# codex-storage/codex-storage-proofs-circuits

Hardware: AMD Instinct MI355X
Metric: Poseidon2-BN254 permutations/sec per GPU; full proof-input witnesses/sec (higher is better)
Workload: dtype u32x9 (29-bit limbs, Montgomery mod BN254 r)

## Files before the change

### codex-storage-proofs-circuits_amd/csrc/internal.hpp

```cpp
#pragma once
#include <hip/hip_runtime.h>

#include <sys/resource.h>
#include <sys/syscall.h>
#include <unistd.h>

#include <condition_variable>
#include <cstdint>
#include <deque>
#include <functional>
#include <memory>
#include <mutex>
#include <string>
#include <thread>
#include <vector>

#include "../../include/codex_p2.h"
#include "workers.hpp"

namespace cp2i {

bool env_decimal(const char* name, uint64_t* value, bool* set);
bool env_keep_trees(int* mode);
size_t mem_limit_bytes();
// ... 135 lines not shown
  void* p = nullptr;
  size_t bytes = 0;
  cp2_ctx* owner = nullptr;
  cp2_ctx* home = nullptr;
  bool borrowed = false;
  DevBuf() = default;
  DevBuf(const DevBuf&) = delete;
  DevBuf& operator=(const DevBuf&) = delete;
  ~DevBuf() { release(); }
  void borrow(void* q, size_t n) {
    release();
    p = q;
    bytes = n;
    borrowed = true;
  }
  void release() {
    if (p && !borrowed) {
      if (owner && owner->stuck) {
      } else if (owner) {
        (void)hipStreamSynchronize(owner->stream);
        if (owner->aux_stream) (void)hipStreamSynchronize(owner->aux_stream);
        if (owner->aux2_stream) (void)hipStreamSynchronize(owner->aux2_stream);
        owner->pool->put(false, p, bytes);
      } else if (!(home && home->stuck)) {
        dev_free(p, bytes);
      }
    }
    p = nullptr;
    bytes = 0;
    owner = nullptr;
    home = nullptr;
    borrowed = false;
  }
  int alloc(cp2_ctx* ctx, size_t n) {
    release();
    if (n == 0) n = 16;
    hipError_t e = dev_malloc(&p, n);
    if (e != hipSuccess) {
      (void)hipGetLastError();
      ctx->pool->trim();
      e = dev_malloc(&p, n);
    }
    if (e != hipSuccess) {
      (void)hipGetLastError();
      p = nullptr;
      ctx->err = std::string("hipMalloc(") + std::to_string(n) + "): " + hipGetErrorString(e);
      return CP2_ERR_ALLOC;
    }
    bytes = n;
    home = ctx;
    return CP2_OK;
  }
  int scratch(cp2_ctx* ctx, size_t n) {
    release();
    size_t got = 0;
    p = ctx->pool->get(false, n, &got);
    if (!p) {
      ctx->err = std::string("device scratch of ") + std::to_string(n) + " bytes: allocation failed";
      return CP2_ERR_ALLOC;
    }
    bytes = got;
    owner = ctx;
    return CP2_OK;
  }
  uint8_t* u8() const { return static_cast<uint8_t*>(p); }
};
// ... 55 lines not shown
```

### codex-storage-proofs-circuits_amd/csrc/proof_many.cpp

```cpp
#include <hip/hip_runtime.h>

#include <fcntl.h>
#include <unistd.h>

#include <algorithm>
#include <cstring>
#include <map>
#include <memory>
#include <string>
#include <vector>

#include "dataset_obj.hpp"
#include "proof_input_obj.hpp"
#include "trees.hpp"

using namespace cp2i;

namespace {

struct Req {
  cp2_dataset* ds = nullptr;
  uint64_t slot = 0;
  uint8_t entropy[32];
  size_t at = 0;
  size_t id = 0;
};

int refuse(cp2_ctx* ctx, size_t i, const std::string& why) {
  ctx->err = "request " + std::to_string(i) + ": " + why;
  return CP2_ERR_INVALID;
}

size_t depth_of(size_t n) { return layer_sizes_of(n).size() - 1; }

bool same_circuit(const cp2_config& a, const cp2_config& b) {
  return a.max_depth == b.max_depth && a.max_log2_nslots == b.max_log2_nslots && a.cell_size == b.cell_size && a.block_size == b.block_size &&
         a.n_samples == b.n_samples;
}

int validate(cp2_ctx* ctx, cp2_dataset* const* ds, const uint64_t* slot_idx, size_t n) {
  for (size_t i = 0; i < n; ++i) {
    const cp2_dataset* d = ds[i];
    if (!d) return refuse(ctx, i, "NULL dataset");
    if (d->ctx != ctx) return refuse(ctx, i, "its dataset belongs to another context");
    const cp2_config& c = d->cfg;
// ... 17 lines not shown
  }
  return CP2_OK;
}

int check_roots(cp2_ctx* ctx, cp2_dataset* const* ds, const uint64_t* slot_idx, size_t n) {
  std::vector<uint64_t> a(n);
  for (size_t i = 0; i < n; ++i)
    a[i] = (uint64_t)reinterpret_cast<uintptr_t>(dataset_roots_dev(ds[i])) + (slot_idx[i] - ds[i]->first_slot) * 32;
  std::vector<uint8_t> got(n * 32);
  DevBuf d_a, d_r;
  CP2_TRY(d_a.scratch(ctx, n * 8));
  CP2_TRY(d_r.scratch(ctx, n * 32));
  CP2_HIP(ctx, hipMemcpyAsync(d_a.p, a.data(), n * 8, hipMemcpyHostToDevice, ctx->stream));
  CP2_HIP(ctx, cp2k::launch_gather_addr(static_cast<const uint64_t*>(d_a.p), n, 32, d_r.p, ctx->stream));
  CP2_HIP(ctx, hipMemcpyAsync(got.data(), d_r.p, n * 32, hipMemcpyDeviceToHost, ctx->stream));
  CP2_HIP(ctx, hipStreamSynchronize(ctx->stream));
  for (size_t i = 0; i < n; ++i)
    if (std::memcmp(&got[i * 32], &ds[i]->dlayers[slot_idx[i] * 32], 32) != 0)
      return refuse(ctx, i, "the root its dataset tree holds for slot " + std::to_string(slot_idx[i]) +
                                " (cp2_dataset_set_roots) differs from the slot's built root");
  return CP2_OK;
}

int prepare(cp2_ctx* ctx, cp2_dataset* const* ds, const uint64_t* slot_idx, size_t n) {
  CP2_TRY(validate(ctx, ds, slot_idx, n));
  CP2_HIP(ctx, hipSetDevice(ctx->device));
  for (size_t i = 0; i < n; ++i)
    if (!ds[i]->have_roots) CP2_TRY(cp2_dataset_set_roots(ds[i], nullptr));
  return check_roots(ctx, ds, slot_idx, n);
}

std::string who(bool named, const Req* r) { return named ? "request " + std::to_string(r->id) + ": " : std::string(); }

int run_pass(cp2_ctx* ctx, const std::vector<const Req*>& rq, size_t n_rf, size_t n_rfile, size_t n_cf, bool named, cp2_proof_input** out) {
  const size_t n = rq.size(), nr = n_rf + n_rfile;
  const cp2_config& c0 = rq[0]->ds->cfg;
  const size_t ns = c0.n_samples, md = (size_t)c0.max_depth, cs = c0.cell_size, bs = c0.block_size, cpb = bs / cs;
  const size_t T = n * ns, R = nr * ns, C = T - R, RF = n_rf * ns, CF = n_cf * ns;
  auto store = std::make_shared<BatchStore>();
  if (T) {
    std::vector<cp2k::ManyReq> reqs(n);
    std::vector<cp2k::TreeGeom> geoms;
    std::map<std::string, uint32_t> geom_of;
    for (size_t j = 0; j < n; ++j) {
      const cp2_dataset* ds = rq[j]->ds;
      cp2k::ManyReq& q = reqs[j];
      std::memset(&q, 0, sizeof q);
      std::memcpy(q.entropy, rq[j]->entropy, 32);
      std::memcpy(q.slot_root, &ds->dlayers[rq[j]->slot * 32], 32);
      q.n_cells = ds->cfg.n_cells;
      q.cpb = cpb;
      if (j < nr) {
        cp2k::TreeGeom g;
        std::memset(&g, 0, sizeof g);
        trees_geom(ds->trees, &g);
        auto it = geom_of.emplace(std::string(reinterpret_cast<const char*>(&g), sizeof g), (uint32_t)geoms.size());
        if (it.second) geoms.push_back(g);
        q.geom = it.first->second;
        q.nodes = (uint64_t)reinterpret_cast<uintptr_t>(ds->trees->nodes.p);
        q.slot = rq[j]->slot - ds->first_slot;
      }
    }
    std::vector<uint64_t> blk(C), gen, cpaths, ctail, ccell;
    std::vector<uint8_t> checks(2 * C * 32);
    PinBuf h_blocks;
    const size_t rows = T * md + T + 2 * C;
    DevBuf d_req, d_geom, d_idx, d_blk, d_addr, d_rows, d_cells, d_gen, d_caddr;
    CP2_TRY(d_req.scratch(ctx, n * sizeof(cp2k::ManyReq)));
    CP2_TRY(d_geom.scratch(ctx, std::max<size_t>(1, geoms.size()) * sizeof(cp2k::TreeGeom)));
    CP2_TRY(d_idx.scratch(ctx, T * 8));
    CP2_TRY(d_blk.scratch(ctx, T * 8));
    CP2_TRY(d_addr.scratch(ctx, rows * 8));
    CP2_TRY(d_rows.scratch(ctx, rows * 32));
    CP2_TRY(d_cells.scratch(ctx, (C * cpb + T) * cs));
    CP2_TRY(store->idx.alloc(ctx, T * 8));
    CP2_TRY(store->paths.alloc(ctx, T * md * 32));
    CP2_TRY(store->leaves.alloc(ctx, T * 32));
    CP2_TRY(store->cells.alloc(ctx, T * cs));
    uint8_t* cells_out = d_cells.u8() + C * cpb * cs;
    uint64_t* addr = static_cast<uint64_t*>(d_addr.p);
    CP2_HIP(ctx, hipMemcpyAsync(d_req.p, reqs.data(), n * sizeof(cp2k::ManyReq), hipMemcpyHostToDevice, ctx->stream));
    if (!geoms.empty())
      CP2_HIP(ctx, hipMemcpyAsync(d_geom.p, geoms.data(), geoms.size() * sizeof(cp2k::TreeGeom), hipMemcpyHostToDevice, ctx->stream));
    CP2_HIP(ctx, cp2k::launch_sample_many(static_cast<const cp2k::ManyReq*>(d_req.p), static_cast<const cp2k::TreeGeom*>(d_geom.p), n,
                                          (uint32_t)ns, (uint32_t)md, static_cast<uint64_t*>(d_idx.p), static_cast<uint64_t*>(d_blk.p), addr,
                                          ctx->stream));
    CP2_HIP(ctx, hipMemcpyAsync(store->idx.p, d_idx.p, T * 8, hipMemcpyDeviceToHost, ctx->stream));
    if (C) CP2_HIP(ctx, hipMemcpyAsync(blk.data(), static_cast<uint64_t*>(d_blk.p) + R, C * 8, hipMemcpyDeviceToHost, ctx->stream));
    CP2_HIP(ctx, hipStreamSynchronize(ctx->stream));
    const uint64_t* idx = static_cast<const uint64_t*>(store->idx.p);

    gen.assign((CF + RF) * 2, 0);
    uint64_t* seeds = gen.data();
    uint64_t* firsts = seeds + CF + RF;
    for (size_t q = 0; q < CF; ++q) {
      const Req* r = rq[nr + q / ns];
      seeds[q] = cp2_slot_seed(r->ds->cfg.seed, r->slot);
      firsts[q] = blk[q] * cpb;
    }
    for (size_t p = 0; p < RF; ++p) {
      const Req* r = rq[p / ns];
      seeds[CF + p] = cp2_slot_seed(r->ds->cfg.seed, r->slot);
      firsts[CF + p] = idx[p];
    }
    if (CF + RF) {
      CP2_TRY(d_gen.scratch(ctx, gen.size() * 8));
      const uint64_t* dg = static_cast<const uint64_t*>(d_gen.p);
      CP2_HIP(ctx, hipMemcpyAsync(d_gen.p, gen.data(), gen.size() * 8, hipMemcpyHostToDevice, ctx->stream));
      CP2_HIP(ctx, cp2k::launch_gen_fake_cells_many(dg, dg + CF + RF, cpb, CF * cpb, cs, d_cells.p, ctx->stream));
      CP2_HIP(ctx, cp2k::launch_gen_fake_cells_many(dg + CF, dg + CF + RF + CF, 1, RF, cs, cells_out, ctx->stream));
    }
    if (C > CF) {
      const size_t n_req_file = (C - CF) / ns;
      CP2_TRY(h_blocks.alloc(ctx, (C - CF) * bs));
      std::vector<std::string> failed(fill_threads(ctx));
      on_threads(fill_threads(ctx), n_req_file, [&](int w, size_t k) {
        const size_t q0 = CF + k * ns;
        const Req* r = rq[nr + q0 / ns];
        const std::string fname = slot_file_name(r->ds->file_base, r->slot);
        const int fd = open(fname.c_str(), O_RDONLY);
        if (fd < 0) { failed[w] = who(named, r) + "slot " + std::to_string(r->slot) + ": " + slot_file_error(fname, 0); return false; }
        int err = 0;
        size_t c = 0;
        for (; c < ns && !err; ++c) err = slot_file_read_rest(fd, h_blocks.u8() + (q0 - CF + c) * bs, bs, blk[q0 + c] * bs);
        close(fd);
        if (err) {
          failed[w] = who(named, r) + "block " + std::to_string(blk[q0 + c - 1]) + " of slot " + std::to_string(r->slot) +
                      ": " + slot_file_error(fname, err);
          return false;
        }
        return true;
      });
      for (const auto& f : failed)
        if (!f.empty()) { ctx->err = f; return CP2_ERR_IO; }
      CP2_HIP(ctx, hipMemcpyAsync(d_cells.u8() + CF * bs, h_blocks.p, (C - CF) * bs, hipMemcpyHostToDevice, ctx->stream));
    }
    cp2_slot_trees* mini = nullptr;
    struct Mini { cp2_slot_trees*& t; ~Mini() { cp2_slot_trees_free(t); } } mini_guard{mini};
    if (C) {
      cpaths.assign(C * md, 0);
      ctail.assign(3 * C, 0);
      ccell.assign(C, 0);
      CP2_TRY(cp2_slot_trees_build_dev(ctx, d_cells.p, C, cs, bs, cpb, &mini));
      const size_t depth_b = depth_of(cpb);
      const uint64_t mb = (uint64_t)reinterpret_cast<uintptr_t>(mini->nodes.p);
      std::vector<uint64_t> rr(depth_b + 1);
      for (size_t q = 0; q < C; ++q) {
        const Req* r = rq[nr + q / ns];
        const cp2_dataset* ds = r->ds;
        const uint64_t ls = r->slot - ds->first_slot, cell = idx[R + q], b = blk[q], in_block = cell % cpb;
        const uint64_t kb = (uint64_t)reinterpret_cast<uintptr_t>(ds->compact.p);
        uint64_t* P = &cpaths[q * md];
        path_rows(mini, q, in_block, depth_b + 1, rr.data());
        for (size_t d = 0; d < depth_b; ++d) P[d] = rr[d] == NO_ROW ? 0 : mb + rr[d] * 32;
        uint64_t j = b, m = ds->cfg.n_cells / cpb;
        for (size_t d = 0; d + 1 < ds->csizes.size(); ++d) {
          const uint64_t sib = j ^ 1;
          P[depth_b + d] = sib < m ? kb + (ds->coff[d] + ls * ds->csizes[d] + sib) * 32 : 0;
          j >>= 1;
          m = (m + 1) >> 1;
        }
        ctail[q] = mb + (q * cpb + in_block) * 32;
        ctail[C + 2 * q] = kb + (ds->coff[0] + ls * ds->csizes[0] + b) * 32;
        ctail[C + 2 * q + 1] = mb + (mini->toff[0] + q) * 32;
        ccell[q] = (uint64_t)reinterpret_cast<uintptr_t>(d_cells.u8()) + (q * cpb + in_block) * cs;
      }
      CP2_TRY(d_caddr.scratch(ctx, C * 8));
      CP2_HIP(ctx, hipMemcpyAsync(addr + R * md, cpaths.data(), C * md * 8, hipMemcpyHostToDevice, ctx->stream));
      CP2_HIP(ctx, hipMemcpyAsync(addr + T * md + R, ctail.data(), 3 * C * 8, hipMemcpyHostToDevice, ctx->stream));
      CP2_HIP(ctx, hipMemcpyAsync(d_caddr.p, ccell.data(), C * 8, hipMemcpyHostToDevice, ctx->stream));
      CP2_HIP(ctx, cp2k::launch_gather_addr(static_cast<const uint64_t*>(d_caddr.p), C, cs, cells_out + R * cs, ctx->stream));
    }
    CP2_HIP(ctx, cp2k::launch_gather_addr(addr, rows, 32, d_rows.p, ctx->stream));
    CP2_HIP(ctx, hipMemcpyAsync(store->paths.p, d_rows.p, T * md * 32, hipMemcpyDeviceToHost, ctx->stream));
    CP2_HIP(ctx, hipMemcpyAsync(store->leaves.p, d_rows.u8() + T * md * 32, T * 32, hipMemcpyDeviceToHost, ctx->stream));
    if (C) CP2_HIP(ctx, hipMemcpyAsync(checks.data(), d_rows.u8() + (T * md + T) * 32, 2 * C * 32, hipMemcpyDeviceToHost, ctx->stream));
    CP2_HIP(ctx, hipMemcpyAsync(store->cells.p, cells_out, T * cs, hipMemcpyDeviceToHost, ctx->stream));
    CP2_HIP(ctx, hipStreamSynchronize(ctx->stream));
    for (size_t q = 0; q < C; ++q)
      if (std::memcmp(&checks[2 * q * 32], &checks[(2 * q + 1) * 32], 32) != 0) {
        const Req* r = rq[nr + q / ns];
        ctx->err = who(named, r) + "block " + std::to_string(blk[q]) + " of slot " + std::to_string(r->slot) +
                   " does not hash to its stored root (slot data changed since the build?)";
        return CP2_ERR_IO;
      }
    if (R > RF) {
      std::vector<std::string> failed(fill_threads(ctx));
      on_threads(fill_threads(ctx), n_rfile, [&](int w, size_t k) {
        const Req* r = rq[n_rf + k];
        const std::string fname = slot_file_name(r->ds->file_base, r->slot);
        const int fd = open(fname.c_str(), O_RDONLY);
        if (fd < 0) { failed[w] = who(named, r) + slot_file_error(fname, 0); return false; }
        int err = 0;
        const size_t p0 = (n_rf + k) * ns;
        for (size_t c = 0; c < ns && !err; ++c) err = read_file_cell(fd, cs, idx[p0 + c], store->cells.u8() + (p0 + c) * cs);
        close(fd);
        if (err) { failed[w] = who(named, r) + slot_file_error(fname, err); return false; }
        return true;
      });
      for (const auto& f : failed)
        if (!f.empty()) { ctx->err = f; return CP2_ERR_IO; }
    }
  }
  std::vector<ProofItem> items(n);
  for (size_t j = 0; j < n; ++j) items[j] = {rq[j]->ds, rq[j]->slot, rq[j]->entropy, &out[rq[j]->at]};
  return proof_inputs_from_store(items.data(), n, store, store->cells.u8());
}

}

int cp2i::prove_requests(cp2_ctx* ctx, cp2_dataset* const* ds, const uint64_t* slot_idx, const uint8_t* entropies, size_t n, size_t at0,
                         bool named, cp2_proof_input** out) {
  for (size_t i = 0; i < n; ++i) out[i] = nullptr;
  if (n == 0) return CP2_OK;
  CP2_HIP(ctx, hipSetDevice(ctx->device));
  std::vector<Req> req(n);
  std::vector<const Req*> res_fake, res_file, cmp_fake, cmp_file, roots_only;
  for (size_t i = 0; i < n; ++i) {
    req[i].ds = ds[i];
    req[i].slot = slot_idx[i];
    req[i].at = i;
    req[i].id = at0 + i;
    canonical_felt(entropies + 32 * i, req[i].entropy);
    const cp2_dataset* d = ds[i];
    (d->trees ? (d->from_file ? res_file : res_fake) : d->tree_mode == 2 ? (d->from_file ? cmp_file : cmp_fake) : roots_only).push_back(&req[i]);
  }
  auto fail = [&](int st) {
    for (size_t i = 0; i < n; ++i) { cp2_proof_input_free(out[i]); out[i] = nullptr; }
    return st;
  };
  for (const Req* r : roots_only) {
    const int st = cp2_proof_inputs_generate_batch(r->ds, &r->slot, 1, r->entropy, &out[r->at]);
    if (st != CP2_OK) {
      ctx->err = who(named, r) + ctx->err;
      return fail(st);
    }
  }
  const cp2_config& c0 = ds[0]->cfg;
  const size_t per_req = std::max<size_t>(1, (size_t)c0.n_samples * c0.block_size);
  const size_t chunk = std::max<size_t>(1, ctx->stage_bytes / per_req);
  std::vector<const Req*> compact(cmp_fake);
  compact.insert(compact.end(), cmp_file.begin(), cmp_file.end());
  const size_t n_res = res_fake.size() + res_file.size();
  size_t c = 0;
  for (bool first = true; first ? n_res + compact.size() > 0 : c < compact.size(); first = false) {
    std::vector<const Req*> rq;
    if (first) {
      rq = res_fake;
      rq.insert(rq.end(), res_file.begin(), res_file.end());
    }
    const size_t c1 = std::min(compact.size(), c + chunk);
    rq.insert(rq.end(), compact.begin() + (long)c, compact.begin() + (long)c1);
    const size_t n_cf = c < cmp_fake.size() ? std::min(c1, cmp_fake.size()) - c : 0;
    const int st = run_pass(ctx, rq, first ? res_fake.size() : 0, first ? res_file.size() : 0, n_cf, named, out);
    if (st != CP2_OK) return fail(st);
    c = c1;
  }
  return CP2_OK;
}

extern "C" int cp2_proof_inputs_generate_many(cp2_ctx* ctx, cp2_dataset* const* ds, const uint64_t* slot_idx, const uint8_t* entropies, size_t n,
                                              cp2_proof_input** out) try {
  if (!ctx) return CP2_ERR_INVALID;
  if (n && (!ds || !slot_idx || !entropies || !out)) {
    ctx->err = "cp2_proof_inputs_generate_many: NULL array";
    return CP2_ERR_INVALID;
  }
  for (size_t i = 0; i < n; ++i) out[i] = nullptr;
  if (n == 0) return CP2_OK;
  CP2_REFUSE_STUCK(ctx);
  CP2_TRY(prepare(ctx, ds, slot_idx, n));
  return prove_requests(ctx, ds, slot_idx, entropies, n, 0, true, out);
} catch (const std::bad_alloc&) {
  return CP2_ERR_ALLOC;
} catch (...) {
  return CP2_ERR_INVALID;
}

extern "C" int cp2_proof_inputs_export_many(cp2_ctx* ctx, cp2_dataset* const* ds, const uint64_t* slot_idx, const uint8_t* entropies, size_t n,
                                            const char* const* paths, int threads, size_t batch, uint64_t* total_bytes) try {
  if (!ctx) return CP2_ERR_INVALID;
  if (n && (!ds || !slot_idx || !entropies)) {
    ctx->err = "cp2_proof_inputs_export_many: NULL array";
    return CP2_ERR_INVALID;
  }
  if (total_bytes) *total_bytes = 0;
  if (n == 0) return CP2_OK;
  CP2_REFUSE_STUCK(ctx);
  CP2_TRY(prepare(ctx, ds, slot_idx, n));
  if (batch == 0) batch = 512;
// ... 38 lines not shown
```

### codex-storage-proofs-circuits_amd/csrc/slot_trees.cpp

```cpp
#include <hip/hip_runtime.h>

#include <fcntl.h>
#include <sys/mman.h>
#include <sys/stat.h>
#include <unistd.h>

#include <algorithm>
#include <atomic>
#include <chrono>
#include <condition_variable>
#include <cstdio>
#include <cstdlib>
#include <cstring>
#include <memory>
#include <mutex>
#include <new>
#include <string>
#include <vector>

#include "trees.hpp"
#include "checksum64.hpp"
#include "fake_turns.hpp"
#include "ingest_turns.hpp"
#include "fill_pipeline.hpp"
// ... 17 lines not shown
}

int aux_stream(cp2_ctx* ctx, hipStream_t* out, int which) {
  hipStream_t& st = which == 2 ? ctx->aux2_stream : ctx->aux_stream;
  if (!st) CP2_HIP(ctx, hipStreamCreateWithFlags(&st, hipStreamNonBlocking));
  *out = st;
  return CP2_OK;
}

std::string slot_file_name(const std::string& base, uint64_t slot) { return fill_slot_file_name(base, slot); }

int trees_check_geometry(size_t cell_size, size_t block_size, size_t n_cells, size_t n_slots) {
  if (cell_size == 0 || block_size == 0 || n_cells == 0 || n_slots == 0) return CP2_ERR_INVALID;
  if (block_size % cell_size != 0) return CP2_ERR_INVALID;
  size_t cpb = block_size / cell_size;
  if (n_cells % cpb != 0) return CP2_ERR_INVALID;
  if (cell_size > ((size_t)1 << 30) || n_cells > ((size_t)1 << 40) || n_slots > ((size_t)1 << 32)) return CP2_ERR_INVALID;
  if ((unsigned __int128)n_cells * n_slots > ((unsigned __int128)1 << 44)) return CP2_ERR_INVALID;
  return CP2_OK;
}

}

cp2i::BuildScratch::~BuildScratch() {
  if (!ctx) return;
  (void)hipSetDevice(ctx->device);
  (void)hipStreamSynchronize(ctx->stream);
  if (ctx->aux_stream) (void)hipStreamSynchronize(ctx->aux_stream);
  if (ctx->aux2_stream) (void)hipStreamSynchronize(ctx->aux2_stream);
}

static int trees_layout(cp2_slot_trees* t, cp2i::DevBuf* borrow_from = nullptr) {
  t->bsizes = layer_sizes_of(t->cpb);
  t->tsizes = layer_sizes_of(t->nblocks);
  if (t->bsizes.size() > (size_t)cp2k::TreeGeom::MAX_LAYERS || t->tsizes.size() > (size_t)cp2k::TreeGeom::MAX_LAYERS) return CP2_ERR_INVALID;
  size_t off = 0;
  t->boff.clear();
  t->toff.clear();
  const size_t nb = t->n_slots * t->nblocks;
  for (size_t k = 0; k < t->bsizes.size(); ++k) {
    t->boff.push_back(off);
    if (k + 1 < t->bsizes.size()) off += nb * t->bsizes[k];
  }
  for (size_t k = 0; k < t->tsizes.size(); ++k) {
    t->toff.push_back(off);
    off += t->n_slots * t->tsizes[k];
  }
  if (borrow_from) {
    if (borrow_from->bytes < off * 32) CP2_TRY(borrow_from->scratch(t->ctx, off * 32));
    t->nodes.borrow(borrow_from->p, off * 32);
    return CP2_OK;
  }
  return t->pooled_nodes ? t->nodes.scratch(t->ctx, off * 32) : t->nodes.alloc(t->ctx, off * 32);
}

size_t cp2i::trees_node_bytes(size_t n_slots, size_t cell_size, size_t block_size, size_t n_cells) {
  const size_t cpb = block_size / cell_size, nblocks = n_cells / cpb;
  size_t per_block = 0, per_slot = 0;
  const std::vector<size_t> b = layer_sizes_of(cpb), t = layer_sizes_of(nblocks);
  for (size_t k = 0; k + 1 < b.size(); ++k) per_block += b[k];
  for (size_t m : t) per_slot += m;
  return n_slots * (nblocks * per_block + per_slot) * 32;
}

void cp2i::trees_geom(const cp2_slot_trees* t, cp2k::TreeGeom* g) {
  std::memset(g, 0, sizeof *g);
  g->nb = (uint32_t)t->bsizes.size();
  g->nt = (uint32_t)t->tsizes.size();
  g->cpb = t->cpb;
  g->nblocks = t->nblocks;
  g->n_cells = t->n_cells;
  for (size_t k = 0; k < t->bsizes.size(); ++k) { g->boff[k] = t->boff[k]; g->bsz[k] = t->bsizes[k]; }
  for (size_t k = 0; k < t->tsizes.size(); ++k) { g->toff[k] = t->toff[k]; g->tsz[k] = t->tsizes[k]; }
}

static cp2_slot_trees* trees_new(cp2_ctx* ctx, size_t n_slots, size_t cell_size, size_t block_size, size_t n_cells) {
  cp2_slot_trees* t = new (std::nothrow) cp2_slot_trees();
  if (!t) return nullptr;
  t->ctx = ctx;
  t->n_slots = n_slots;
  t->cell_size = cell_size;
  t->block_size = block_size;
  t->n_cells = n_cells;
  t->cpb = block_size / cell_size;
  t->nblocks = n_cells / t->cpb;
  return t;
}

static int trees_build_layers(cp2_slot_trees* t, size_t s0, size_t s1, hipStream_t st) {
  cp2_ctx* ctx = t->ctx;
  uint8_t* base = t->nodes.u8();
  const size_t ns = s1 - s0, nb = ns * t->nblocks;
  for (size_t k = 0; k + 1 < t->bsizes.size(); ++k)
    CP2_HIP(ctx, cp2k::launch_compress_layer(base + (t->boff[k] + s0 * t->nblocks * t->bsizes[k]) * 32,
                                             base + (t->boff[k + 1] + s0 * t->nblocks * t->bsizes[k + 1]) * 32, t->bsizes[k], nb,
// ... 141 lines not shown
namespace {
bool unit_geometry_ok(uint64_t units_per_slot, size_t cell_size, size_t block_size, size_t cells_per_unit) {
  if (!is_pow2(units_per_slot) || cell_size == 0 || block_size < cell_size) return false;
  const size_t nb = cells_per_unit / (block_size / cell_size);
  return nb >= 2 && is_pow2(nb);
}
}
extern "C" int cp2_slot_trees_build_fake_units(cp2_ctx* ctx, uint64_t dataset_seed, uint64_t units_per_slot, uint64_t first_unit,
                                               size_t n_units, size_t cell_size, size_t block_size, size_t cells_per_unit,
                                               cp2_slot_trees** out) try {
  if (!ctx || !out || units_per_slot == 0) return CP2_ERR_INVALID;
  CP2_TRY(trees_check_geometry(cell_size, block_size, cells_per_unit, n_units));
  if (units_per_slot > 1 && !unit_geometry_ok(units_per_slot, cell_size, block_size, cells_per_unit)) return CP2_ERR_INVALID;
  return trees_build_fake(ctx, dataset_seed, first_unit, n_units, cell_size, block_size, cells_per_unit, 0, nullptr, out, units_per_slot);
} catch (const std::bad_alloc&) {
  return CP2_ERR_ALLOC;
} catch (...) {
  return CP2_ERR_INVALID;
}

extern "C" int cp2_slot_trees_build_file_units(cp2_ctx* ctx, const char* file_base, uint64_t units_per_slot, uint64_t first_unit,
                                               size_t n_units, size_t cell_size, size_t block_size, size_t cells_per_unit,
                                               cp2_slot_trees** out) try {
  if (!ctx || !out || !file_base || units_per_slot == 0 || cell_size > SLOT_FILE_MAX_CELL) return CP2_ERR_INVALID;
  CP2_TRY(trees_check_geometry(cell_size, block_size, cells_per_unit, n_units));
  if (units_per_slot > 1 && !unit_geometry_ok(units_per_slot, cell_size, block_size, cells_per_unit)) return CP2_ERR_INVALID;
  return trees_build_files(ctx, file_base, first_unit, n_units, cell_size, block_size, cells_per_unit, 0, nullptr, out, units_per_slot);
} catch (const std::bad_alloc&) {
  return CP2_ERR_ALLOC;
} catch (...) {
  return CP2_ERR_INVALID;
}

extern "C" int cp2_slot_trees_build_dev(cp2_ctx* ctx, const void* d_cells, size_t n_slots, size_t cell_size,
                                        size_t block_size, size_t n_cells, cp2_slot_trees** out) try {
  if (!ctx || !out || !d_cells) return CP2_ERR_INVALID;
  *out = nullptr;
  CP2_REFUSE_STUCK(ctx);
  CP2_TRY(trees_check_geometry(cell_size, block_size, n_cells, n_slots));
  CP2_HIP(ctx, hipSetDevice(ctx->device));
  std::unique_ptr<cp2_slot_trees> t(trees_new(ctx, n_slots, cell_size, block_size, n_cells));
  if (!t) return CP2_ERR_ALLOC;
  t->src = CellSrc::Dev;
  t->d_cells = static_cast<const uint8_t*>(d_cells);
  CP2_TRY(trees_layout(t.get()));
  CP2_HIP(ctx, cp2k::launch_hash_cells(d_cells, cell_size, n_slots * n_cells, t->nodes.p, ctx->stream));
  CP2_TRY(trees_build_layers(t.get(), 0, n_slots, ctx->stream));
  *out = t.release();
  return CP2_OK;
} catch (const std::bad_alloc&) {
  return CP2_ERR_ALLOC;
} catch (...) {
  return CP2_ERR_INVALID;
}

namespace {

size_t env_size(const char* name, size_t dflt) {
  const char* v = std::getenv(name);
  if (!v || !*v) return dflt;
  char* end = nullptr;
  unsigned long long x = std::strtoull(v, &end, 10);
  return (end && *end == 0 && x > 0) ? (size_t)x : dflt;
}

struct IngestPipe {
  static constexpr int MAX_DEPTH = 8;
  static constexpr size_t DIRECT_ALIGN = 4096;
  size_t cell_multiple = 1;
  cp2_ctx* ctx = nullptr;
  hipStream_t copy = nullptr;
  int pin_depth = 0, dev_depth = 0;
  PinBuf pinned[MAX_DEPTH];
  DevBuf dev[MAX_DEPTH];
  hipEvent_t copied[MAX_DEPTH] = {};
  hipEvent_t uploaded[MAX_DEPTH] = {};
  hipEvent_t hashed[MAX_DEPTH] = {};
  size_t chunk = 0;
  size_t cap_bytes = 0;
  size_t turn = 0;
  size_t pin_turn = 0;
  int threads = 1;
// ... 994 lines not shown
```

### codex-storage-proofs-circuits_amd/csrc/trees.hpp

```cpp
#pragma once
#include <functional>
#include <string>
#include <vector>

#include "internal.hpp"
#include "kernels.hpp"
#include "fill_pipeline.hpp"

enum class CellSrc { Fake, Dev, Host, File };

struct cp2_slot_trees {
  cp2_ctx* ctx = nullptr;
  size_t n_slots = 0, cell_size = 0, block_size = 0, n_cells = 0, cpb = 0, nblocks = 0;
  std::vector<size_t> bsizes, tsizes;
  std::vector<size_t> boff, toff;
  cp2i::DevBuf nodes;
  CellSrc src = CellSrc::Fake;
  uint64_t dataset_seed = 0, first_slot = 0;
  uint64_t units_per_slot = 1;
  bool pooled_nodes = false;
  const uint8_t* d_cells = nullptr;
  const uint8_t* h_cells = nullptr;
  std::string file_base;
};

namespace cp2i {

constexpr uint64_t NO_ROW = ~0ULL;

using SlotsDone = std::function<int(cp2_slot_trees* t, size_t s0, size_t s1, hipStream_t st)>;

struct BuildScratch {
  cp2_ctx* ctx = nullptr;
  DevBuf stage[2], nodes[2];
  hipStream_t tail_stream = nullptr;
  std::shared_ptr<void> file_pipe;
  ~BuildScratch();
};

int trees_check_geometry(size_t cell_size, size_t block_size, size_t n_cells, size_t n_slots);
int trees_build_fake(cp2_ctx* ctx, uint64_t dataset_seed, uint64_t first_slot, size_t n_slots, size_t cell_size, size_t block_size,
                     size_t n_cells, size_t group, const SlotsDone& done, cp2_slot_trees** out, uint64_t units_per_slot = 1,
                     bool pooled_nodes = false, BuildScratch* scratch = nullptr, int node_slot = 0);
int trees_build_files(cp2_ctx* ctx, const std::string& base, uint64_t first_slot, size_t n_slots, size_t cell_size,
                      size_t block_size, size_t n_cells, size_t group, const SlotsDone& done, cp2_slot_trees** out,
                      uint64_t units_per_slot = 1, bool pooled_nodes = false, BuildScratch* scratch = nullptr, int node_slot = 0);
int trees_build_file_list(cp2_ctx* ctx, const std::string* names, size_t n_names, size_t cell_size, size_t block_size, size_t n_cells,
                          size_t group, const SlotsDone& done, cp2_slot_trees** out, bool pooled_nodes = false,
                          BuildScratch* scratch = nullptr, int node_slot = 0);
inline int trees_build_file_list(cp2_ctx* ctx, const std::vector<std::string>& names, size_t cell_size, size_t block_size, size_t n_cells,
                                 size_t group, const SlotsDone& done, cp2_slot_trees** out, bool pooled_nodes = false,
                                 BuildScratch* scratch = nullptr, int node_slot = 0) {
  return trees_build_file_list(ctx, names.data(), names.size(), cell_size, block_size, n_cells, group, done, out, pooled_nodes, scratch, node_slot);
}
size_t trees_node_bytes(size_t n_slots, size_t cell_size, size_t block_size, size_t n_cells);
void trees_geom(const cp2_slot_trees* t, cp2k::TreeGeom* g);
void path_rows(const cp2_slot_trees* t, size_t slot, uint64_t cell, size_t max_depth, uint64_t* rows);
int trees_paths_multi(cp2_slot_trees* t, const uint64_t* slot_idx, const uint64_t* cell_idx, size_t n, size_t max_depth, uint8_t* out, uint8_t* leaf_hashes);
std::string slot_file_name(const std::string& base, uint64_t slot);
bool is_pow2(uint64_t x);

struct KeptMeta {
  uint64_t n_slots = 0, cell_size = 0, block_size = 0, n_cells = 0, src = 0, dataset_seed = 0, first_slot = 0, mode = 0;
  std::string file_base;
};
int kept_save(cp2_ctx* ctx, const char* path, const KeptMeta& meta, const void* d_buf, size_t bytes);
int kept_load(cp2_ctx* ctx, const char* path, const KeptMeta& want, void* d_buf, size_t bytes);

struct FileStamp;
int cache_restamp(const char* path, uint64_t n_items, size_t cell_size, size_t block_size, size_t n_cells, uint64_t first_item,
                  uint64_t units_per_slot, const std::string& base, const std::vector<FileStamp>& written, size_t* restamped, std::string* err);

int dataset_own_roots_in_place(cp2_dataset* ds, bool* ok);

struct ScrubSrc {
  bool from_file = false;
  std::string file_base;
  uint64_t seed = 0;
  size_t cell_size = 0, block_size = 0, n_cells = 0;
  uint64_t units_per_slot = 1;
};
int scrub_items(cp2_ctx* ctx, const ScrubSrc& src, uint64_t item0, uint64_t n, int level, const uint8_t* kept, size_t kstride, size_t cap,
                std::vector<uint64_t>& bad, uint64_t* n_bad);
int dataset_scrub_level(const cp2_dataset* ds);
int dataset_scrub(cp2_dataset* ds, uint64_t first_slot, uint64_t n, int level, size_t cap, std::vector<uint64_t>& bad, uint64_t* n_bad);

bool stream_serial();

// ... 9 lines not shown
```

Before: 777.0 million.

## Pack proof-input pass scratch into one per-call device and pinned host block

Replaces the many per-pass device scratch allocations and pageable host vectors with a single pooled device block and a pinned host staging block, both sized once per call from a shared layout and reused across passes. Address tables are now built on the host before upload and sent in one copy instead of several. The mini tree over sampled blocks now builds only the block roots rather than an upper tree, and it writes into the preallocated node region. The aim is to cut allocator calls, pageable copies and upload count. The cost is more complex layout bookkeeping and larger upfront allocations.

```diff
diff --git a/codex-storage-proofs-circuits_amd/csrc/internal.hpp b/codex-storage-proofs-circuits_amd/csrc/internal.hpp
--- a/codex-storage-proofs-circuits_amd/csrc/internal.hpp
+++ b/codex-storage-proofs-circuits_amd/csrc/internal.hpp
@@ -191,6 +191,13 @@
     home = nullptr;
     borrowed = false;
   }
+  void release_idle() {
+    if (p && owner && !borrowed && !owner->stuck) {
+      owner->pool->put(false, p, bytes);
+      p = nullptr;
+    }
+    release();
+  }
   int alloc(cp2_ctx* ctx, size_t n) {
     release();
     if (n == 0) n = 16;
diff --git a/codex-storage-proofs-circuits_amd/csrc/pass_layout.hpp b/codex-storage-proofs-circuits_amd/csrc/pass_layout.hpp
--- /dev/null
+++ b/codex-storage-proofs-circuits_amd/csrc/pass_layout.hpp
@@ -0,0 +1,76 @@
+#pragma once
+#include <cstddef>
+
+namespace cp2i {
+
+struct PassDims {
+  size_t n = 0, nr = 0, ns = 0, md = 0, G = 0, cpb = 1, cs = 0;
+  size_t req_bytes = 0, geom_bytes = 0;
+};
+
+struct PassRegion {
+  size_t off = 0, bytes = 0, elem_align = 1;
+};
+
+constexpr size_t PASS_ALIGN = 256;
+
+inline size_t pass_block_tree_rows(size_t cpb) {
+  size_t rows = 0, m = cpb;
+  bool bottom = true;
+  for (;;) {
+    rows += m;
+    if (m == 1 && !bottom) return rows;
+    m = (m + 1) / 2;
+    bottom = false;
+  }
+}
+
+struct PassLayout {
+  size_t T = 0, R = 0, C = 0, rows = 0;
+  size_t geoms_off = 0;
+  size_t caddr_at = 0, gen_at = 0;
+  size_t up2_first = 0, up2_count = 0;
+  enum { D_UP1, D_IDX, D_BLK, D_TABLES, D_ROWS, D_CELLS, D_NODES, D_COUNT };
+  enum { H_UP1, H_UP2, H_BLK, H_CHECKS, H_COUNT };
+  PassRegion dev[D_COUNT], host[H_COUNT];
+  size_t dev_total = 0, host_total = 0;
+};
+
+inline size_t pass_place(PassRegion* r, size_t n_regions) {
+  size_t off = 0;
+  for (size_t i = 0; i < n_regions; ++i) {
+    r[i].off = off;
+    off = (off + r[i].bytes + PASS_ALIGN - 1) / PASS_ALIGN * PASS_ALIGN;
+  }
+  return off;
+}
+
+inline PassLayout pass_layout(const PassDims& d) {
+  PassLayout L;
+  L.T = d.n * d.ns;
+  L.R = d.nr * d.ns;
+  L.C = L.T - L.R;
+  L.rows = L.T * d.md + L.T + 2 * L.C;
+  L.geoms_off = d.n * d.req_bytes;
+  L.caddr_at = L.rows;
+  L.gen_at = L.rows + L.C;
+  L.up2_first = L.R * d.md;
+  L.up2_count = L.gen_at + 2 * d.G - L.up2_first;
+  const size_t up1 = L.geoms_off + (d.nr ? d.nr : 1) * d.geom_bytes;
+  L.dev[PassLayout::D_UP1] = {0, up1, 16};
+  L.dev[PassLayout::D_IDX] = {0, L.T * 8, 8};
+  L.dev[PassLayout::D_BLK] = {0, L.T * 8, 8};
+  L.dev[PassLayout::D_TABLES] = {0, (L.gen_at + 2 * d.G) * 8, 8};
+  L.dev[PassLayout::D_ROWS] = {0, L.rows * 32, 16};
+  L.dev[PassLayout::D_CELLS] = {0, (L.C * d.cpb + L.T) * d.cs, 16};
+  L.dev[PassLayout::D_NODES] = {0, L.C * pass_block_tree_rows(d.cpb) * 32, 16};
+  L.dev_total = pass_place(L.dev, PassLayout::D_COUNT);
+  L.host[PassLayout::H_UP1] = {0, up1, 16};
+  L.host[PassLayout::H_UP2] = {0, L.up2_count * 8, 8};
+  L.host[PassLayout::H_BLK] = {0, L.C * 8, 8};
+  L.host[PassLayout::H_CHECKS] = {0, 2 * L.C * 32, 1};
+  L.host_total = pass_place(L.host, PassLayout::H_COUNT);
+  return L;
+}
+
+}
diff --git a/codex-storage-proofs-circuits_amd/csrc/proof_many.cpp b/codex-storage-proofs-circuits_amd/csrc/proof_many.cpp
--- a/codex-storage-proofs-circuits_amd/csrc/proof_many.cpp
+++ b/codex-storage-proofs-circuits_amd/csrc/proof_many.cpp
@@ -11,6 +11,7 @@
 #include <vector>
 
 #include "dataset_obj.hpp"
+#include "pass_layout.hpp"
 #include "proof_input_obj.hpp"
 #include "trees.hpp"
 
@@ -94,15 +95,47 @@
 
 std::string who(bool named, const Req* r) { return named ? "request " + std::to_string(r->id) + ": " : std::string(); }
 
-int run_pass(cp2_ctx* ctx, const std::vector<const Req*>& rq, size_t n_rf, size_t n_rfile, size_t n_cf, bool named, cp2_proof_input** out) {
+struct CallScratch {
+  PinBuf h_stage, h_blocks;
+  DevBuf d_block;
+};
+
+static_assert(sizeof(cp2k::ManyReq) == 112 && sizeof(cp2k::TreeGeom) == 1312 && sizeof(cp2k::ManyReq) % alignof(cp2k::TreeGeom) == 0,
+              "pass_layout.hpp's up1 region: descriptor and geometry sizes");
+
+PassDims dims_of(const cp2_config& c0, size_t n, size_t n_rf, size_t n_rfile, size_t n_cf) {
+  PassDims d;
+  d.n = n;
+  d.nr = n_rf + n_rfile;
+  d.ns = c0.n_samples;
+  d.md = (size_t)c0.max_depth;
+  d.G = (n_cf + n_rf) * d.ns;
+  d.cs = c0.cell_size;
+  d.cpb = c0.block_size / c0.cell_size;
+  d.req_bytes = sizeof(cp2k::ManyReq);
+  d.geom_bytes = sizeof(cp2k::TreeGeom);
+  return d;
+}
+
+int run_pass_body(cp2_ctx* ctx, const std::vector<const Req*>& rq, size_t n_rf, size_t n_rfile, size_t n_cf, bool named, CallScratch& sc,
+                  cp2_proof_input** out, StageTimer& trace) {
   const size_t n = rq.size(), nr = n_rf + n_rfile;
   const cp2_config& c0 = rq[0]->ds->cfg;
   const size_t ns = c0.n_samples, md = (size_t)c0.max_depth, cs = c0.cell_size, bs = c0.block_size, cpb = bs / cs;
-  const size_t T = n * ns, R = nr * ns, C = T - R, RF = n_rf * ns, CF = n_cf * ns;
+  const PassLayout L = pass_layout(dims_of(c0, n, n_rf, n_rfile, n_cf));
+  const size_t T = L.T, R = L.R, C = L.C, RF = n_rf * ns, CF = n_cf * ns, G = CF + RF, rows = L.rows;
   auto store = std::make_shared<BatchStore>();
+  struct Drain { cp2_ctx* ctx; bool armed; ~Drain() { if (armed && !ctx->stuck) (void)hipStreamSynchronize(ctx->stream); } } drain{ctx, false};
   if (T) {
-    std::vector<cp2k::ManyReq> reqs(n);
-    std::vector<cp2k::TreeGeom> geoms;
+    if (L.dev_total > sc.d_block.bytes || L.host_total > sc.h_stage.bytes || (C - CF) * bs > sc.h_blocks.bytes) {
+      ctx->err = "proof-input pass: the call's scratch does not hold this pass";
+      return CP2_ERR_INVALID;
+    }
+    auto dev = [&](int r) { return sc.d_block.u8() + L.dev[r].off; };
+    auto host = [&](int r) { return sc.h_stage.u8() + L.host[r].off; };
+    cp2k::ManyReq* reqs = reinterpret_cast<cp2k::ManyReq*>(host(PassLayout::H_UP1));
+    cp2k::TreeGeom* geoms = reinterpret_cast<cp2k::TreeGeom*>(host(PassLayout::H_UP1) + L.geoms_off);
+    size_t n_geoms = 0;
     std::map<std::string, uint32_t> geom_of;
     for (size_t j = 0; j < n; ++j) {
       const cp2_dataset* ds = rq[j]->ds;
@@ -116,45 +149,46 @@
         cp2k::TreeGeom g;
         std::memset(&g, 0, sizeof g);
         trees_geom(ds->trees, &g);
-        auto it = geom_of.emplace(std::string(reinterpret_cast<const char*>(&g), sizeof g), (uint32_t)geoms.size());
-        if (it.second) geoms.push_back(g);
+        auto it = geom_of.emplace(std::string(reinterpret_cast<const char*>(&g), sizeof g), (uint32_t)n_geoms);
+        if (it.second) geoms[n_geoms++] = g;
         q.geom = it.first->second;
         q.nodes = (uint64_t)reinterpret_cast<uintptr_t>(ds->trees->nodes.p);
         q.slot = rq[j]->slot - ds->first_slot;
       }
     }
-    std::vector<uint64_t> blk(C), gen, cpaths, ctail, ccell;
-    std::vector<uint8_t> checks(2 * C * 32);
-    PinBuf h_blocks;
-    const size_t rows = T * md + T + 2 * C;
-    DevBuf d_req, d_geom, d_idx, d_blk, d_addr, d_rows, d_cells, d_gen, d_caddr;
-    CP2_TRY(d_req.scratch(ctx, n * sizeof(cp2k::ManyReq)));
-    CP2_TRY(d_geom.scratch(ctx, std::max<size_t>(1, geoms.size()) * sizeof(cp2k::TreeGeom)));
-    CP2_TRY(d_idx.scratch(ctx, T * 8));
-    CP2_TRY(d_blk.scratch(ctx, T * 8));
-    CP2_TRY(d_addr.scratch(ctx, rows * 8));
-    CP2_TRY(d_rows.scratch(ctx, rows * 32));
-    CP2_TRY(d_cells.scratch(ctx, (C * cpb + T) * cs));
+    trace.lap("pass: descriptors");
     CP2_TRY(store->idx.alloc(ctx, T * 8));
     CP2_TRY(store->paths.alloc(ctx, T * md * 32));
     CP2_TRY(store->leaves.alloc(ctx, T * 32));
     CP2_TRY(store->cells.alloc(ctx, T * cs));
-    uint8_t* cells_out = d_cells.u8() + C * cpb * cs;
-    uint64_t* addr = static_cast<uint64_t*>(d_addr.p);
-    CP2_HIP(ctx, hipMemcpyAsync(d_req.p, reqs.data(), n * sizeof(cp2k::ManyReq), hipMemcpyHostToDevice, ctx->stream));
-    if (!geoms.empty())
-      CP2_HIP(ctx, hipMemcpyAsync(d_geom.p, geoms.data(), geoms.size() * sizeof(cp2k::TreeGeom), hipMemcpyHostToDevice, ctx->stream));
-    CP2_HIP(ctx, cp2k::launch_sample_many(static_cast<const cp2k::ManyReq*>(d_req.p), static_cast<const cp2k::TreeGeom*>(d_geom.p), n,
-                                          (uint32_t)ns, (uint32_t)md, static_cast<uint64_t*>(d_idx.p), static_cast<uint64_t*>(d_blk.p), addr,
-                                          ctx->stream));
-    CP2_HIP(ctx, hipMemcpyAsync(store->idx.p, d_idx.p, T * 8, hipMemcpyDeviceToHost, ctx->stream));
-    if (C) CP2_HIP(ctx, hipMemcpyAsync(blk.data(), static_cast<uint64_t*>(d_blk.p) + R, C * 8, hipMemcpyDeviceToHost, ctx->stream));
+    uint64_t* d_idx = reinterpret_cast<uint64_t*>(dev(PassLayout::D_IDX));
+    uint64_t* d_blk = reinterpret_cast<uint64_t*>(dev(PassLayout::D_BLK));
+    uint64_t* addr = reinterpret_cast<uint64_t*>(dev(PassLayout::D_TABLES));
+    uint8_t* d_rows = dev(PassLayout::D_ROWS);
+    uint8_t* d_cells = dev(PassLayout::D_CELLS);
+    uint8_t* cells_out = d_cells + C * cpb * cs;
+    const uint64_t* blk = reinterpret_cast<const uint64_t*>(host(PassLayout::H_BLK));
+    const uint8_t* checks = host(PassLayout::H_CHECKS);
+    trace.lap("pass: store buffers");
+    drain.armed = true;
+    CP2_HIP(ctx, hipMemcpyAsync(dev(PassLayout::D_UP1), reqs, L.geoms_off + n_geoms * sizeof(cp2k::TreeGeom), hipMemcpyHostToDevice, ctx->stream));
+    CP2_HIP(ctx, cp2k::launch_sample_many(reinterpret_cast<const cp2k::ManyReq*>(dev(PassLayout::D_UP1)),
+                                          reinterpret_cast<const cp2k::TreeGeom*>(dev(PassLayout::D_UP1) + L.geoms_off), n, (uint32_t)ns,
+                                          (uint32_t)md, d_idx, d_blk, addr, ctx->stream));
+    CP2_HIP(ctx, hipMemcpyAsync(store->idx.p, d_idx, T * 8, hipMemcpyDeviceToHost, ctx->stream));
+    if (C) CP2_HIP(ctx, hipMemcpyAsync(host(PassLayout::H_BLK), d_blk + R, C * 8, hipMemcpyDeviceToHost, ctx->stream));
     CP2_HIP(ctx, hipStreamSynchronize(ctx->stream));
     const uint64_t* idx = static_cast<const uint64_t*>(store->idx.p);
-
-    gen.assign((CF + RF) * 2, 0);
-    uint64_t* seeds = gen.data();
-    uint64_t* firsts = seeds + CF + RF;
+    trace.lap("pass: sample + first synchronise");
+
+    uint64_t* up2 = reinterpret_cast<uint64_t*>(host(PassLayout::H_UP2));
+    auto table = [&](size_t at) -> uint64_t& { return up2[at - L.up2_first]; };
+    for (size_t p = 0; p < R; ++p) {
+      const cp2k::ManyReq& q = reqs[p / ns];
+      table(T * md + p) = q.nodes + (q.slot * rq[p / ns]->ds->trees->n_cells + idx[p]) * 32;
+    }
+    uint64_t* seeds = &table(L.gen_at);
+    uint64_t* firsts = seeds + G;
     for (size_t q = 0; q < CF; ++q) {
       const Req* r = rq[nr + q / ns];
       seeds[q] = cp2_slot_seed(r->ds->cfg.seed, r->slot);
@@ -165,16 +199,45 @@
       seeds[CF + p] = cp2_slot_seed(r->ds->cfg.seed, r->slot);
       firsts[CF + p] = idx[p];
     }
-    if (CF + RF) {
-      CP2_TRY(d_gen.scratch(ctx, gen.size() * 8));
-      const uint64_t* dg = static_cast<const uint64_t*>(d_gen.p);
-      CP2_HIP(ctx, hipMemcpyAsync(d_gen.p, gen.data(), gen.size() * 8, hipMemcpyHostToDevice, ctx->stream));
-      CP2_HIP(ctx, cp2k::launch_gen_fake_cells_many(dg, dg + CF + RF, cpb, CF * cpb, cs, d_cells.p, ctx->stream));
-      CP2_HIP(ctx, cp2k::launch_gen_fake_cells_many(dg + CF, dg + CF + RF + CF, 1, RF, cs, cells_out, ctx->stream));
+    cp2_slot_trees* mini = nullptr;
+    struct Mini { cp2_slot_trees*& t; ~Mini() { cp2_slot_trees_free(t); } } mini_guard{mini};
+    if (C) {
+      CP2_TRY(trees_dev_new(ctx, d_cells, C, cs, bs, cpb, true, dev(PassLayout::D_NODES), L.dev[PassLayout::D_NODES].bytes, &mini));
+      const size_t depth_b = depth_of(cpb);
+      const uint64_t mb = (uint64_t)reinterpret_cast<uintptr_t>(mini->nodes.p);
+      std::vector<uint64_t> rr(depth_b);
+      for (size_t q = 0; q < C; ++q) {
+        const Req* r = rq[nr + q / ns];
+        const cp2_dataset* ds = r->ds;
+        const uint64_t ls = r->slot - ds->first_slot, cell = idx[R + q], b = blk[q], in_block = cell % cpb;
+        const uint64_t kb = (uint64_t)reinterpret_cast<uintptr_t>(ds->compact.p);
+        uint64_t* P = &table((R + q) * md);
+        path_rows(mini, q, in_block, depth_b, rr.data());
+        for (size_t d = 0; d < md; ++d) P[d] = 0;
+        for (size_t d = 0; d < depth_b; ++d) P[d] = rr[d] == NO_ROW ? 0 : mb + rr[d] * 32;
+        uint64_t j = b, m = ds->cfg.n_cells / cpb;
+        for (size_t d = 0; d + 1 < ds->csizes.size(); ++d) {
+          const uint64_t sib = j ^ 1;
+          P[depth_b + d] = sib < m ? kb + (ds->coff[d] + ls * ds->csizes[d] + sib) * 32 : 0;
+          j >>= 1;
+          m = (m + 1) >> 1;
+        }
+        table(T * md + R + q) = mb + (q * cpb + in_block) * 32;
+        table(T * md + T + 2 * q) = kb + (ds->coff[0] + ls * ds->csizes[0] + b) * 32;
+        table(T * md + T + 2 * q + 1) = mb + (mini->toff[0] + q) * 32;
+        table(L.caddr_at + q) = (uint64_t)reinterpret_cast<uintptr_t>(d_cells) + (q * cpb + in_block) * cs;
+      }
+    }
+    trace.lap("pass: address tables");
+    if (L.up2_count) CP2_HIP(ctx, hipMemcpyAsync(addr + L.up2_first, up2, L.up2_count * 8, hipMemcpyHostToDevice, ctx->stream));
+    if (G) {
+      const uint64_t* dg = addr + L.gen_at;
+      CP2_HIP(ctx, cp2k::launch_gen_fake_cells_many(dg, dg + G, cpb, CF * cpb, cs, d_cells, ctx->stream));
+      CP2_HIP(ctx, cp2k::launch_gen_fake_cells_many(dg + CF, dg + G + CF, 1, RF, cs, cells_out, ctx->stream));
     }
     if (C > CF) {
       const size_t n_req_file = (C - CF) / ns;
-      CP2_TRY(h_blocks.alloc(ctx, (C - CF) * bs));
+      uint8_t* h_blocks = sc.h_blocks.u8();
       std::vector<std::string> failed(fill_threads(ctx));
       on_threads(fill_threads(ctx), n_req_file, [&](int w, size_t k) {
         const size_t q0 = CF + k * ns;
@@ -184,7 +247,7 @@
         if (fd < 0) { failed[w] = who(named, r) + "slot " + std::to_string(r->slot) + ": " + slot_file_error(fname, 0); return false; }
         int err = 0;
         size_t c = 0;
-        for (; c < ns && !err; ++c) err = slot_file_read_rest(fd, h_blocks.u8() + (q0 - CF + c) * bs, bs, blk[q0 + c] * bs);
+        for (; c < ns && !err; ++c) err = slot_file_read_rest(fd, h_blocks + (q0 - CF + c) * bs, bs, blk[q0 + c] * bs);
         close(fd);
         if (err) {
           failed[w] = who(named, r) + "block " + std::to_string(blk[q0 + c - 1]) + " of slot " + std::to_string(r->slot) +
@@ -195,50 +258,22 @@
       });
       for (const auto& f : failed)
         if (!f.empty()) { ctx->err = f; return CP2_ERR_IO; }
-      CP2_HIP(ctx, hipMemcpyAsync(d_cells.u8() + CF * bs, h_blocks.p, (C - CF) * bs, hipMemcpyHostToDevice, ctx->stream));
-    }
-    cp2_slot_trees* mini = nullptr;
-    struct Mini { cp2_slot_trees*& t; ~Mini() { cp2_slot_trees_free(t); } } mini_guard{mini};
+      CP2_HIP(ctx, hipMemcpyAsync(d_cells + CF * bs, h_blocks, (C - CF) * bs, hipMemcpyHostToDevice, ctx->stream));
+    }
+    trace.lap("pass: generate / read + upload");
     if (C) {
-      cpaths.assign(C * md, 0);
-      ctail.assign(3 * C, 0);
-      ccell.assign(C, 0);
-      CP2_TRY(cp2_slot_trees_build_dev(ctx, d_cells.p, C, cs, bs, cpb, &mini));
-      const size_t depth_b = depth_of(cpb);
-      const uint64_t mb = (uint64_t)reinterpret_cast<uintptr_t>(mini->nodes.p);
-      std::vector<uint64_t> rr(depth_b + 1);
-      for (size_t q = 0; q < C; ++q) {
-        const Req* r = rq[nr + q / ns];
-        const cp2_dataset* ds = r->ds;
-        const uint64_t ls = r->slot - ds->first_slot, cell = idx[R + q], b = blk[q], in_block = cell % cpb;
-        const uint64_t kb = (uint64_t)reinterpret_cast<uintptr_t>(ds->compact.p);
-        uint64_t* P = &cpaths[q * md];
-        path_rows(mini, q, in_block, depth_b + 1, rr.data());
-        for (size_t d = 0; d < depth_b; ++d) P[d] = rr[d] == NO_ROW ? 0 : mb + rr[d] * 32;
-        uint64_t j = b, m = ds->cfg.n_cells / cpb;
-        for (size_t d = 0; d + 1 < ds->csizes.size(); ++d) {
-          const uint64_t sib = j ^ 1;
-          P[depth_b + d] = sib < m ? kb + (ds->coff[d] + ls * ds->csizes[d] + sib) * 32 : 0;
-          j >>= 1;
-          m = (m + 1) >> 1;
-        }
-        ctail[q] = mb + (q * cpb + in_block) * 32;
-        ctail[C + 2 * q] = kb + (ds->coff[0] + ls * ds->csizes[0] + b) * 32;
-        ctail[C + 2 * q + 1] = mb + (mini->toff[0] + q) * 32;
-        ccell[q] = (uint64_t)reinterpret_cast<uintptr_t>(d_cells.u8()) + (q * cpb + in_block) * cs;
-      }
-      CP2_TRY(d_caddr.scratch(ctx, C * 8));
-      CP2_HIP(ctx, hipMemcpyAsync(addr + R * md, cpaths.data(), C * md * 8, hipMemcpyHostToDevice, ctx->stream));
-      CP2_HIP(ctx, hipMemcpyAsync(addr + T * md + R, ctail.data(), 3 * C * 8, hipMemcpyHostToDevice, ctx->stream));
-      CP2_HIP(ctx, hipMemcpyAsync(d_caddr.p, ccell.data(), C * 8, hipMemcpyHostToDevice, ctx->stream));
-      CP2_HIP(ctx, cp2k::launch_gather_addr(static_cast<const uint64_t*>(d_caddr.p), C, cs, cells_out + R * cs, ctx->stream));
-    }
-    CP2_HIP(ctx, cp2k::launch_gather_addr(addr, rows, 32, d_rows.p, ctx->stream));
-    CP2_HIP(ctx, hipMemcpyAsync(store->paths.p, d_rows.p, T * md * 32, hipMemcpyDeviceToHost, ctx->stream));
-    CP2_HIP(ctx, hipMemcpyAsync(store->leaves.p, d_rows.u8() + T * md * 32, T * 32, hipMemcpyDeviceToHost, ctx->stream));
-    if (C) CP2_HIP(ctx, hipMemcpyAsync(checks.data(), d_rows.u8() + (T * md + T) * 32, 2 * C * 32, hipMemcpyDeviceToHost, ctx->stream));
+      CP2_TRY(trees_dev_enqueue(mini));
+      CP2_HIP(ctx, cp2k::launch_gather_addr(addr + L.caddr_at, C, cs, cells_out + R * cs, ctx->stream));
+    }
+    trace.lap("pass: hash + layers enqueued");
+    CP2_HIP(ctx, cp2k::launch_gather_addr(addr, rows, 32, d_rows, ctx->stream));
+    CP2_HIP(ctx, hipMemcpyAsync(store->paths.p, d_rows, T * md * 32, hipMemcpyDeviceToHost, ctx->stream));
+    CP2_HIP(ctx, hipMemcpyAsync(store->leaves.p, d_rows + T * md * 32, T * 32, hipMemcpyDeviceToHost, ctx->stream));
+    if (C) CP2_HIP(ctx, hipMemcpyAsync(host(PassLayout::H_CHECKS), d_rows + (T * md + T) * 32, 2 * C * 32, hipMemcpyDeviceToHost, ctx->stream));
     CP2_HIP(ctx, hipMemcpyAsync(store->cells.p, cells_out, T * cs, hipMemcpyDeviceToHost, ctx->stream));
     CP2_HIP(ctx, hipStreamSynchronize(ctx->stream));
+    drain.armed = false;
+    trace.lap("pass: gathers + downloads + second synchronise");
     for (size_t q = 0; q < C; ++q)
       if (std::memcmp(&checks[2 * q * 32], &checks[(2 * q + 1) * 32], 32) != 0) {
         const Req* r = rq[nr + q / ns];
@@ -266,7 +301,15 @@
   }
   std::vector<ProofItem> items(n);
   for (size_t j = 0; j < n; ++j) items[j] = {rq[j]->ds, rq[j]->slot, rq[j]->entropy, &out[rq[j]->at]};
-  return proof_inputs_from_store(items.data(), n, store, store->cells.u8());
+  const int st = proof_inputs_from_store(items.data(), n, store, store->cells.u8());
+  trace.lap("pass: checks + objects");
+  return st;
+}
+
+int run_pass(cp2_ctx* ctx, const std::vector<const Req*>& rq, size_t n_rf, size_t n_rfile, size_t n_cf, bool named, CallScratch& sc,
+             cp2_proof_input** out) {
+  StageTimer trace;
+  return run_pass_body(ctx, rq, n_rf, n_rfile, n_cf, named, sc, out, trace);
 }
 
 }
@@ -304,20 +347,44 @@
   std::vector<const Req*> compact(cmp_fake);
   compact.insert(compact.end(), cmp_file.begin(), cmp_file.end());
   const size_t n_res = res_fake.size() + res_file.size();
+  if (n_res + compact.size() == 0) return CP2_OK;
+  std::vector<size_t> sizes;
+  for (size_t c = 0; c < compact.size() || sizes.empty(); c += chunk) sizes.push_back(std::min(chunk, compact.size() - c));
+  StageTimer trace;
+  CallScratch sc;
+  size_t dev_bytes = 0, host_bytes = 0, file_bytes = 0;
+  {
+    size_t c = 0;
+    for (size_t k = 0; k < sizes.size(); ++k) {
+      const size_t c1 = c + sizes[k], n_cf = c < cmp_fake.size() ? std::min(c1, cmp_fake.size()) - c : 0;
+      const PassLayout L = pass_layout(dims_of(c0, (k ? 0 : n_res) + sizes[k], k ? 0 : res_fake.size(), k ? 0 : res_file.size(), n_cf));
+      dev_bytes = std::max(dev_bytes, L.dev_total);
+      host_bytes = std::max(host_bytes, L.host_total);
+      file_bytes = std::max(file_bytes, (sizes[k] - n_cf) * c0.n_samples * c0.block_size);
+      c = c1;
+    }
+  }
+  if (host_bytes) CP2_TRY(sc.h_stage.alloc(ctx, host_bytes));
+  if (file_bytes) CP2_TRY(sc.h_blocks.alloc(ctx, file_bytes));
+  if (dev_bytes) CP2_TRY(sc.d_block.scratch(ctx, dev_bytes));
+  trace.lap("pass: the call's scratch blocks");
   size_t c = 0;
-  for (bool first = true; first ? n_res + compact.size() > 0 : c < compact.size(); first = false) {
+  for (size_t k = 0; k < sizes.size(); ++k) {
     std::vector<const Req*> rq;
-    if (first) {
+    if (k == 0) {
       rq = res_fake;
       rq.insert(rq.end(), res_file.begin(), res_file.end());
     }
-    const size_t c1 = std::min(compact.size(), c + chunk);
+    const size_t c1 = c + sizes[k];
     rq.insert(rq.end(), compact.begin() + (long)c, compact.begin() + (long)c1);
     const size_t n_cf = c < cmp_fake.size() ? std::min(c1, cmp_fake.size()) - c : 0;
-    const int st = run_pass(ctx, rq, first ? res_fake.size() : 0, first ? res_file.size() : 0, n_cf, named, out);
+    const int st = run_pass(ctx, rq, k ? 0 : res_fake.size(), k ? 0 : res_file.size(), n_cf, named, sc, out);
     if (st != CP2_OK) return fail(st);
     c = c1;
   }
+  StageTimer trace_release;
+  sc.d_block.release_idle();
+  trace_release.lap("pass: the call's scratch release");
   return CP2_OK;
 }
 
diff --git a/codex-storage-proofs-circuits_amd/csrc/slot_trees.cpp b/codex-storage-proofs-circuits_amd/csrc/slot_trees.cpp
--- a/codex-storage-proofs-circuits_amd/csrc/slot_trees.cpp
+++ b/codex-storage-proofs-circuits_amd/csrc/slot_trees.cpp
@@ -73,7 +73,7 @@
 
 static int trees_layout(cp2_slot_trees* t, cp2i::DevBuf* borrow_from = nullptr) {
   t->bsizes = layer_sizes_of(t->cpb);
-  t->tsizes = layer_sizes_of(t->nblocks);
+  t->tsizes = t->block_roots_only ? std::vector<size_t>{t->nblocks} : layer_sizes_of(t->nblocks);
   if (t->bsizes.size() > (size_t)cp2k::TreeGeom::MAX_LAYERS || t->tsizes.size() > (size_t)cp2k::TreeGeom::MAX_LAYERS) return CP2_ERR_INVALID;
   size_t off = 0;
   t->boff.clear();
@@ -92,16 +92,21 @@
     t->nodes.borrow(borrow_from->p, off * 32);
     return CP2_OK;
   }
+  if (t->nodes.borrowed) return CP2_OK;
   return t->pooled_nodes ? t->nodes.scratch(t->ctx, off * 32) : t->nodes.alloc(t->ctx, off * 32);
 }
 
-size_t cp2i::trees_node_bytes(size_t n_slots, size_t cell_size, size_t block_size, size_t n_cells) {
+size_t cp2i::trees_node_rows(size_t n_slots, size_t cell_size, size_t block_size, size_t n_cells, bool block_roots_only) {
   const size_t cpb = block_size / cell_size, nblocks = n_cells / cpb;
   size_t per_block = 0, per_slot = 0;
   const std::vector<size_t> b = layer_sizes_of(cpb), t = layer_sizes_of(nblocks);
   for (size_t k = 0; k + 1 < b.size(); ++k) per_block += b[k];
-  for (size_t m : t) per_slot += m;
-  return n_slots * (nblocks * per_block + per_slot) * 32;
+  if (block_roots_only) per_slot = nblocks;
+  else for (size_t m : t) per_slot += m;
+  return n_slots * (nblocks * per_block + per_slot);
+}
+size_t cp2i::trees_node_bytes(size_t n_slots, size_t cell_size, size_t block_size, size_t n_cells) {
+  return trees_node_rows(n_slots, cell_size, block_size, n_cells, false) * 32;
 }
 
 void cp2i::trees_geom(const cp2_slot_trees* t, cp2k::TreeGeom* g) {
@@ -309,9 +314,8 @@
   return CP2_ERR_INVALID;
 }
 
-extern "C" int cp2_slot_trees_build_dev(cp2_ctx* ctx, const void* d_cells, size_t n_slots, size_t cell_size,
-                                        size_t block_size, size_t n_cells, cp2_slot_trees** out) try {
-  if (!ctx || !out || !d_cells) return CP2_ERR_INVALID;
+int cp2i::trees_dev_new(cp2_ctx* ctx, const void* d_cells, size_t n_slots, size_t cell_size, size_t block_size, size_t n_cells,
+                        bool block_roots_only, void* nodes, size_t nodes_bytes, cp2_slot_trees** out) {
   *out = nullptr;
   CP2_REFUSE_STUCK(ctx);
   CP2_TRY(trees_check_geometry(cell_size, block_size, n_cells, n_slots));
@@ -320,11 +324,32 @@
   if (!t) return CP2_ERR_ALLOC;
   t->src = CellSrc::Dev;
   t->d_cells = static_cast<const uint8_t*>(d_cells);
+  t->block_roots_only = block_roots_only;
+  if (nodes) {
+    if (trees_node_rows(n_slots, cell_size, block_size, n_cells, block_roots_only) * 32 > nodes_bytes) {
+      ctx->err = "device trees: the node buffer handed in is too small";
+      return CP2_ERR_INVALID;
+    }
+    t->nodes.borrow(nodes, nodes_bytes);
+  }
   CP2_TRY(trees_layout(t.get()));
-  CP2_HIP(ctx, cp2k::launch_hash_cells(d_cells, cell_size, n_slots * n_cells, t->nodes.p, ctx->stream));
-  CP2_TRY(trees_build_layers(t.get(), 0, n_slots, ctx->stream));
   *out = t.release();
   return CP2_OK;
+}
+
+int cp2i::trees_dev_enqueue(cp2_slot_trees* t) {
+  cp2_ctx* ctx = t->ctx;
+  CP2_HIP(ctx, cp2k::launch_hash_cells(t->d_cells, t->cell_size, t->n_slots * t->n_cells, t->nodes.p, ctx->stream));
+  return trees_build_layers(t, 0, t->n_slots, ctx->stream);
+}
+
+extern "C" int cp2_slot_trees_build_dev(cp2_ctx* ctx, const void* d_cells, size_t n_slots, size_t cell_size,
+                                        size_t block_size, size_t n_cells, cp2_slot_trees** out) try {
+  if (!ctx || !out || !d_cells) return CP2_ERR_INVALID;
+  CP2_TRY(trees_dev_new(ctx, d_cells, n_slots, cell_size, block_size, n_cells, false, nullptr, 0, out));
+  const int st = trees_dev_enqueue(*out);
+  if (st != CP2_OK) { cp2_slot_trees_free(*out); *out = nullptr; }
+  return st;
 } catch (const std::bad_alloc&) {
   return CP2_ERR_ALLOC;
 } catch (...) {
diff --git a/codex-storage-proofs-circuits_amd/csrc/trees.hpp b/codex-storage-proofs-circuits_amd/csrc/trees.hpp
--- a/codex-storage-proofs-circuits_amd/csrc/trees.hpp
+++ b/codex-storage-proofs-circuits_amd/csrc/trees.hpp
@@ -18,6 +18,7 @@
   CellSrc src = CellSrc::Fake;
   uint64_t dataset_seed = 0, first_slot = 0;
   uint64_t units_per_slot = 1;
+  bool block_roots_only = false;
   bool pooled_nodes = false;
   const uint8_t* d_cells = nullptr;
   const uint8_t* h_cells = nullptr;
@@ -54,6 +55,10 @@
   return trees_build_file_list(ctx, names.data(), names.size(), cell_size, block_size, n_cells, group, done, out, pooled_nodes, scratch, node_slot);
 }
 size_t trees_node_bytes(size_t n_slots, size_t cell_size, size_t block_size, size_t n_cells);
+size_t trees_node_rows(size_t n_slots, size_t cell_size, size_t block_size, size_t n_cells, bool block_roots_only);
+int trees_dev_new(cp2_ctx* ctx, const void* d_cells, size_t n_slots, size_t cell_size, size_t block_size, size_t n_cells,
+                  bool block_roots_only, void* nodes, size_t nodes_bytes, cp2_slot_trees** out);
+int trees_dev_enqueue(cp2_slot_trees* t);
 void trees_geom(const cp2_slot_trees* t, cp2k::TreeGeom* g);
 void path_rows(const cp2_slot_trees* t, size_t slot, uint64_t cell, size_t max_depth, uint64_t* rows);
 int trees_paths_multi(cp2_slot_trees* t, const uint64_t* slot_idx, const uint64_t* cell_idx, size_t n, size_t max_depth, uint8_t* out, uint8_t* leaf_hashes);
```

Result: no change. 776.1 million (-0.1%).
